# sqlp/sedumi

Hardware: AMD Instinct MI355X
Metric: IPM iters/sec (ADA' form+factor+solve) (higher is better)
Workload: dtype f64; 1 GPU; control07.mat: examples/control07.mat (BASELINE.json configs[1]), m=666, nnz(At)=107940, nnz(ADA')=443556, nnz(L)=222111; unit = getada1+2+3, blkchol, 4x(fwblkslv,./d,bwblkslv); parallelism=single GPU

## Files before the change

### sedumi_amd/csrc/sdm_ada.hip

```cpp
#include "sdm_plan.h"
#include <algorithm>
#include <cmath>
#include <cstdlib>

namespace sdm {

void ada_build(sdm_plan *P, sdm_int N, sdm_int m, const sdm_int *Ajc, const sdm_int *Air, const double *Apr,
               const sdm_int *Ajc_psd, sdm_int lpN, sdm_int lorN, const sdm_int *lorNL, sdm_int sdpN,
               sdm_int rsdpN, const sdm_int *sdpNL, const sdm_int *qblkstart, const sdm_int *psd_blkstart,
               const sdm_int *Qjc, const sdm_int *Qir, const sdm_int *ADAjc, const sdm_int *ADAir) {
  AdaPlan &A = P->ada;
  A.N = N; A.m = m; A.nnzA = Ajc[m]; A.lpN = lpN; A.lorN = lorN; A.sdpN = sdpN; A.rsdpN = rsdpN;
  A.ic_n.release(); A.ufac.release();
  if (A.nnzA >= (sdm_int)1 << 31 || N >= (sdm_int)1 << 31) throw std::runtime_error("At too large for 32-bit row indices");
  (void)lorNL;
  A.nlq = sdpN > 0 ? psd_blkstart[0] : N;
  if (lorN > 0 && qblkstart[lorN] != A.nlq && sdpN > 0) throw std::runtime_error("qblkstart / psd_blkstart mismatch");
  {
    std::vector<int> code((size_t)A.nlq, -1);
    for (sdm_int r = lpN; r < lpN + lorN && r < A.nlq; r++) code[r] = (int)(-2 - (r - lpN));
    for (sdm_int k = 0; k < lorN; k++)
      for (sdm_int r = qblkstart[k]; r < qblkstart[k + 1] && r < A.nlq; r++) code[r] = (int)k;
    A.dsqr_code.upload(code);
  }
// ... 443 lines not shown
  const int task = order ? order[blockIdx.x] : blockIdx.x + task0;
  const int n = T.t_n[task], nslot = T.t_nslot[task], ulen = T.t_ulen[task];
  const int herm = T.t_herm[task];
  const int64_t slot0 = T.t_slotptr[task], tend = T.t_end[task];
  const double *D = udsqr + T.t_udoff[task];
  const double *Di = D + (int64_t)n * n;
  const int *U = T.u_pos + T.t_uoff[task];
  double *z = zbuf + T.t_zoff[task];
  const int64_t rowbase = T.psd_start[T.t_blk[task]];
  const int tid = threadIdx.x, bs = blockDim.x;
  const int wave = tid >> 6, lane = tid & 63, nw = bs >> 6;
  int CC = ldsY / (n * (herm ? 4 : 2)); if (CC < 1) CC = 1; if (CC > nslot) CC = nslot;
  double *Yi = Y + (int64_t)CC * n;
  double *Dl = Y + (int64_t)(herm ? 2 : 1) * CC * n;
  double *Dli = Dl + (int64_t)CC * n;
  double *nzx = Y + ldsY;
  int *nzr = (int *)(nzx + nzcap);
  __shared__ int scol[256];
  const int64_t nzb = T.s_nzptr[slot0];
  const bool staged = tend - nzb <= nzcap;
  if (staged)
    for (int64_t u = nzb + tid; u < tend; u += bs) { nzx[u - nzb] = T.Apr[u]; nzr[u - nzb] = (int)(T.Air[u] - rowbase); }
  constexpr int S1_TREG = 6;
  int rreg[S1_TREG], creg[S1_TREG];
  double zreg[S1_TREG];
  const int nreg = herm ? 0 : min(ulen, S1_TREG * bs);
  if (!herm) {
#pragma unroll
    for (int k = 0; k < S1_TREG; k++) {
      const int q = U[min(tid + k * bs, max(ulen - 1, 0))];
      creg[k] = q / n; rreg[k] = q - creg[k] * n; zreg[k] = 0.0;
    }
  }
  for (int c0 = 0; c0 < nslot; c0 += CC) {
    const int cc = min(CC, nslot - c0);
    for (int t = tid; t < min(cc, 256); t += bs) scol[t] = T.s_col[slot0 + c0 + t];
    __syncthreads();
    const bool flat = cc < nw;
    for (int t = flat ? 0 : wave; t < cc; t += flat ? 1 : nw) {
      const int64_t sb = T.s_nzptr[slot0 + c0 + t];
      const int64_t se = (c0 + t + 1 < nslot) ? T.s_nzptr[slot0 + c0 + t + 1] : tend;
      const int sc = t < 256 ? scol[t] : T.s_col[slot0 + c0 + t];
      const int part = sc >= n ? 1 : 0, col = sc - part * n;
      const int sub0 = part * n * n + col * n;
      if (!herm && !flat && n <= 256) {
        double a4[4] = {0.0, 0.0, 0.0, 0.0}, d4[4];
        int i4[4];
#pragma unroll
        for (int k = 0; k < 4; k++) { i4[k] = min(lane + 64 * k, n - 1); d4[k] = D[(int64_t)col * n + i4[k]]; }
        for (int64_t u = sb; u < se; u++) {
          const int rx = (staged ? nzr[u - nzb] : (int)(T.Air[u] - rowbase)) - sub0;
          const double x = staged ? nzx[u - nzb] : T.Apr[u];
          double dr[4];
#pragma unroll
          for (int k = 0; k < 4; k++) dr[k] = D[(int64_t)rx * n + i4[k]];
#pragma unroll
          for (int k = 0; k < 4; k++) a4[k] += x * dr[k];
        }
#pragma unroll
        for (int k = 0; k < 4; k++)
          if (lane + 64 * k < n) { Y[t * n + lane + 64 * k] = a4[k]; Dl[t * n + lane + 64 * k] = d4[k]; }
        continue;
      }
      for (int i = flat ? tid : lane; i < n; i += flat ? bs : 64) {
        double ar = 0.0, ai = 0.0;
        for (int64_t u = sb; u < se; u++) {
          const int rx = (staged ? nzr[u - nzb] : (int)(T.Air[u] - rowbase)) - sub0;
          const double x = staged ? nzx[u - nzb] : T.Apr[u], dr = D[(int64_t)rx * n + i];
          if (!herm) ar += x * dr;
          else {
            const double di = Di[(int64_t)rx * n + i];
            if (part) { ar -= x * di; ai += x * dr; } else { ar += x * dr; ai += x * di; }
          }
        }
        Y[t * n + i] = ar;
        Dl[t * n + i] = D[(int64_t)col * n + i];
        if (herm) { Yi[t * n + i] = ai; Dli[t * n + i] = -Di[(int64_t)col * n + i]; }
      }
    }
    __syncthreads();
    if (!herm) {
      double sreg[S1_TREG];
#pragma unroll
      for (int k = 0; k < S1_TREG; k++) sreg[k] = 0.0;
#pragma unroll 1
      for (int t = 0; t < cc; t++) {
        const double *Yt = Y + t * n, *Dt = Dl + t * n;
#pragma unroll
        for (int k = 0; k < S1_TREG; k++) sreg[k] += Yt[rreg[k]] * Dt[creg[k]] + Yt[creg[k]] * Dt[rreg[k]];
      }
#pragma unroll
      for (int k = 0; k < S1_TREG; k++) zreg[k] += sreg[k] / 2;
    }
    for (int u = nreg + tid; u < ulen; u += bs) {
      int q = U[u];
      const int zpart = q >= n * n ? 1 : 0;
      q -= zpart * n * n;
      const int c = q / n, r = q - c * n;
      double v;
      if (!herm) {
        double a1 = 0.0, a2 = 0.0;
        for (int t = 0; t < cc; t++) {
          a1 += Y[t * n + r] * Dl[t * n + c];
          a2 += Y[t * n + c] * Dl[t * n + r];
        }
        v = (a1 + a2) / 2;
      } else {
        double rrc = 0.0, irc = 0.0, rcr = 0.0, icr = 0.0;
        for (int t = 0; t < cc; t++) {
          const double drc = Dl[t * n + c], dic = Dli[t * n + c], drr = Dl[t * n + r], dir = Dli[t * n + r];
          const double yr_r = Y[t * n + r], yi_r = Yi[t * n + r], yr_c = Y[t * n + c], yi_c = Yi[t * n + c];
          rrc += yr_r * drc - yi_r * dic; irc += yr_r * dic + yi_r * drc;
          rcr += yr_c * drr - yi_c * dir; icr += yr_c * dir + yi_c * drr;
        }
        v = zpart ? (irc - icr) / 2 : (rrc + rcr) / 2;
      }
      if (c0 == 0) z[u] = v; else z[u] += v;
    }
    __syncthreads();
  }
  if (!herm && R2.ada && ulen <= S1_TREG * bs) {
    double *zl = Y;
#pragma unroll
    for (int k = 0; k < S1_TREG; k++) if (tid + k * bs < ulen) zl[tid + k * bs] = zreg[k];
    __syncthreads();
    const int j = R2.t_col[task], kblk = T.t_blk[task];
    const int ipj = R2.invperm ? R2.invperm[j] : 0;
    for (int64_t e = R2.ADAjc[j] + tid; e < R2.ADAjc[j + 1]; e += bs) {
      const int i = R2.ADAir[e];
      if (R2.invperm && R2.invperm[i] > ipj) continue;
      double acc = 0.0, aabs = 0.0;
      int64_t p = R2.Ajc_psd[i];
      const int64_t pe = R2.Ajc[i + 1];
      for (; p + 4 <= pe; p += 4) {
        double x[4]; int b[4], u[4];
#pragma unroll
        for (int q = 0; q < 4; q++) { x[q] = R2.Apr[p + q]; b[q] = R2.Ablk[p + q]; u[q] = R2.Aupos[p + q]; }
#pragma unroll
        for (int q = 0; q < 4; q++) if (b[q] == kblk) { const double term = x[q] * zl[u[q]]; acc += term; aabs += fabs(term); }
      }
      for (; p < pe; p++) if (R2.Ablk[p] == kblk) { const double term = R2.Apr[p] * zl[R2.Aupos[p]]; acc += term; aabs += fabs(term); }
      const double base = R2.ada[e];
      R2.ada[e] = base + acc;
      if (i == j) R2.absd[j] = base + aabs;
    }
    return;
  }
  if (!herm) {
#pragma unroll
    for (int k = 0; k < S1_TREG; k++) if (tid + k * bs < ulen) z[tid + k * bs] = zreg[k];
  }
}

__global__ void __launch_bounds__(64 * S1_WAVES, 4)
k_psd_stage1_mfma(Stage1Tab T, const double *udsqr, double *zbuf, int task0, const int *order, double *zero_ptr, long long zero_n) {
  SDM_DYN_SMEM(smem);
  for (long long i = (long long)blockIdx.x * blockDim.x + threadIdx.x; i < zero_n; i += (long long)gridDim.x * blockDim.x) zero_ptr[i] = 0.0;
  const int task = order ? order[blockIdx.x] : blockIdx.x + task0;
  const int n = T.t_n[task], nslot = T.t_nslot[task], ulen = T.t_ulen[task];
  const int np = (n + 15) & ~15, nt = np >> 4, ntile = nt * nt;
  double *Yl = (double *)smem;
  double *Dl = Yl + S1_KC * np;
  double *Zl = (double *)smem;
  const int64_t slot0 = T.t_slotptr[task], tend = T.t_end[task];
  const double *D = udsqr + T.t_udoff[task];
  double *z = zbuf + T.t_zoff[task];
  const int64_t rowbase = T.psd_start[T.t_blk[task]];
  const int tid = threadIdx.x, bs = blockDim.x;
  const int wave = SDM_UNIFORM_INT(tid >> 6), lane = tid & 63, nw = bs >> 6;
  const int li = lane & 15, lk = lane >> 4;
  sdm_double4 acc[S1_MAXT];
  for (int x = 0; x < S1_MAXT; x++) for (int r = 0; r < 4; r++) acc[x][r] = 0.0;
  __shared__ double nzx[S1_NZ];
  __shared__ int nzr[S1_NZ];
  __shared__ int sbeg[S1_MAXN + 1], scol[S1_MAXN];
  SDM_PHASE_BEGIN();
  const int64_t nzb = T.s_nzptr[slot0];
  const bool staged = tend - nzb <= S1_NZ && nslot <= S1_MAXN;
  if (staged) {
    for (int64_t u = nzb + tid; u < tend; u += bs) { nzx[u - nzb] = T.Apr[u]; nzr[u - nzb] = (int)(T.Air[u] - rowbase); }
    for (int t = tid; t <= nslot; t += bs) sbeg[t] = (int)((t < nslot ? T.s_nzptr[slot0 + t] : tend) - nzb);
    for (int t = tid; t < nslot; t += bs) scol[t] = T.s_col[slot0 + t];
  }
  __syncthreads();
  SDM_PHASE(0);
  for (int c0 = 0; c0 < nslot; c0 += S1_KC) {
    const int cc = min(S1_KC, nslot - c0);
    for (int t = wave; t < S1_KC; t += nw) {
      if (t < cc) {
        int sb, se, col;
        if (staged) { sb = sbeg[c0 + t]; se = sbeg[c0 + t + 1]; col = scol[c0 + t]; }
        else {
          sb = (int)(T.s_nzptr[slot0 + c0 + t] - nzb);
          se = (int)(((c0 + t + 1 < nslot) ? T.s_nzptr[slot0 + c0 + t + 1] : tend) - nzb);
          col = T.s_col[slot0 + c0 + t];
        }
        for (int i = lane; i < np; i += 64) {
          double a = 0.0;
          if (i < n) {
            if (staged) {
              int u = sb;
              for (; u + 4 <= se; u += 4) {
                const double d0 = D[(int64_t)(nzr[u] - col * n) * n + i], d1 = D[(int64_t)(nzr[u + 1] - col * n) * n + i];
                const double d2 = D[(int64_t)(nzr[u + 2] - col * n) * n + i], d3 = D[(int64_t)(nzr[u + 3] - col * n) * n + i];
                a += nzx[u] * d0; a += nzx[u + 1] * d1; a += nzx[u + 2] * d2; a += nzx[u + 3] * d3;
              }
              for (; u < se; u++) a += nzx[u] * D[(int64_t)(nzr[u] - col * n) * n + i];
            } else {
              for (int64_t u = nzb + sb; u < nzb + se; u++) a += T.Apr[u] * D[(int64_t)((int)(T.Air[u] - rowbase) - col * n) * n + i];
            }
          }
          Yl[t * np + i] = a;
          Dl[t * np + i] = i < n ? D[(int64_t)col * n + i] : 0.0;
        }
      } else {
        for (int i = lane; i < np; i += 64) { Yl[t * np + i] = 0.0; Dl[t * np + i] = 0.0; }
      }
    }
    SDM_PHASE(1);
    __syncthreads();
    SDM_PHASE(2);
    for (int x = 0; x < S1_MAXT; x++) {
      const int tile = wave + x * nw;
      if (tile < ntile) {
        const int I = tile / nt, J = tile - I * nt;
#pragma unroll 4
        for (int q = 0; q < S1_KC / 4; q++) {
          const double a = Yl[(4 * q + lk) * np + I * 16 + li];
          const double b = Dl[(4 * q + lk) * np + J * 16 + li];
          acc[x] = SDM_MFMA_F64_16x16x4(a, b, acc[x]);
        }
      }
    }
    SDM_PHASE(3);
    __syncthreads();
    SDM_PHASE(4);
  }
  for (int x = 0; x < S1_MAXT; x++) {
    const int tile = wave + x * nw;
    if (tile < ntile) {
      const int I = tile / nt, J = tile - I * nt;
      for (int r = 0; r < 4; r++) Zl[(I * 16 + lk + 4 * r) * np + J * 16 + li] = acc[x][r];
    }
  }
  __syncthreads();
  SDM_PHASE(5);
  const int *RC = T.u_rc + T.t_uoff[task];
  for (int u0 = 0; u0 < ulen; u0 += 8 * bs) {
    int rc[8];
#pragma unroll
    for (int x = 0; x < 8; x++) rc[x] = RC[min(u0 + x * bs + tid, ulen - 1)];
#pragma unroll
    for (int x = 0; x < 8; x++) {
      const int u = u0 + x * bs + tid;
      const int r = rc[x] >> 16, c = rc[x] & 0xffff;
      if (u < ulen) z[u] = (Zl[r * np + c] + Zl[c * np + r]) / 2;
    }
  }
  SDM_PHASE(6);
#if defined(SDM_PHASES) && !defined(SDM_EMU)
  if (tid == 0) { atomicAdd(&sdm_phase_acc[30], 1ull); if (n > 40) atomicAdd(&sdm_phase_acc[31], 1ull); }
#endif
}

__global__ void __launch_bounds__(256)
k_psd_stage2(double *ada, double *absd, const int64_t *ADAjc, const int *ADAir, const int64_t *Ajc,
             const int64_t *Ajc_psd, const double *Apr, const int *Ablk, const int *Aupos,
             const int64_t *c_taskptr, const int *t_blk, const int64_t *t_zoff, const int64_t *c_zlen, const double *zbuf,
             const int *invperm, int nblk, int thread_per_row, int jbase, int zlds) {
  SDM_DYN_SMEM(smem);
  long long *zo = (long long *)smem;
  double *zl = (double *)(zo + nblk);
  const int j = blockIdx.x + jbase;
  const int tid = threadIdx.x, bs = blockDim.x;
  const int64_t tb0 = c_taskptr[j], te0 = c_taskptr[j + 1];
  const bool jhas = te0 > tb0;
  const int64_t z0 = jhas ? t_zoff[tb0] : 0;
  const int64_t zlen = c_zlen[j];
  for (int k = tid; k < nblk; k += bs) zo[k] = -1;
  __syncthreads();
  for (int64_t t = tb0 + tid; t < te0; t += bs) zo[t_blk[t]] = t_zoff[t] - z0;
  const bool staged = thread_per_row && jhas && zlen <= zlds;
  if (staged)
    for (int64_t u = tid; u < zlen; u += bs) zl[u] = zbuf[z0 + u];
  __syncthreads();
  const double *zsrc = staged ? zl : zbuf + z0;
  const int ipj = invperm ? invperm[j] : 0;
  if (thread_per_row) {
    for (int64_t e = ADAjc[j] + tid; e < ADAjc[j + 1]; e += bs) {
      const int i = ADAir[e];
      if (invperm && invperm[i] > ipj) continue;
      double acc = 0.0, aabs = 0.0;
      if (jhas) {
        int64_t t = Ajc_psd[i];
        const int64_t te = Ajc[i + 1];
        for (; t + 4 <= te; t += 4) {
          double x[4]; int b[4], u[4];
#pragma unroll
          for (int q = 0; q < 4; q++) { x[q] = Apr[t + q]; b[q] = Ablk[t + q]; u[q] = Aupos[t + q]; }
#pragma unroll
          for (int q = 0; q < 4; q++) {
            const long long off = zo[b[q]];
            if (off >= 0) { const double term = x[q] * zsrc[off + u[q]]; acc += term; aabs += fabs(term); }
          }
        }
        for (; t < te; t++) {
          const long long off = zo[Ablk[t]];
          if (off >= 0) { const double term = Apr[t] * zsrc[off + Aupos[t]]; acc += term; aabs += fabs(term); }
        }
      }
      const double base = ada[e];
      ada[e] = base + acc;
      if (i == j) absd[j] = jhas ? base + aabs : 0.0;
    }
  } else {
    const int wave = tid >> 6, lane = tid & 63, nw = bs >> 6;
    for (int64_t e = ADAjc[j] + wave; e < ADAjc[j + 1]; e += nw) {
      const int i = ADAir[e];
      if (invperm && invperm[i] > ipj) continue;
      double acc = 0.0, aabs = 0.0;
      if (jhas)
        for (int64_t t = Ajc_psd[i] + lane; t < Ajc[i + 1]; t += 64) {
          const long long off = zo[Ablk[t]];
          if (off >= 0) { const double term = Apr[t] * zsrc[off + Aupos[t]]; acc += term; aabs += fabs(term); }
        }
      for (int off = 32; off > 0; off >>= 1) { acc += __shfl_down(acc, off); aabs += __shfl_down(aabs, off); }
      if (lane == 0) {
        const double base = ada[e];
        ada[e] = base + acc;
        if (i == j) absd[j] = jhas ? base + aabs : 0.0;
      }
    }
  }
}

constexpr int S1_DIRECT_MAXNZ = 2;
constexpr int DIRECT_JB = 8;
__global__ void __launch_bounds__(256)
k_psd_direct_cols(double *ada, double *absd, const int64_t *ADAjc, const int64_t *Ajc, const int64_t *Ajc_psd, const double *Apr,
                  const int *Air, const int *Ablk, const int64_t *c_taskptr, const int *t_blk, const int *t_n, const int64_t *t_udoff,
                  const int64_t *t_slotptr, const int64_t *s_nzptr, const int64_t *t_end, const int64_t *psd_start, const double *udsqr,
                  int nblk, int jbase, int jend, int m, int base_zero) {
  SDM_DYN_SMEM(smem);
  const int per_i = 2 * nblk + 2 * S1_DIRECT_MAXNZ * nblk + 2, per_ll = 2 * nblk, per_d = S1_DIRECT_MAXNZ * nblk;
  int *bn_all = (int *)smem;
  long long *ll_all = (long long *)(bn_all + DIRECT_JB * (per_i + (per_i & 1)));
  double *bx_all = (double *)(ll_all + DIRECT_JB * per_ll);
  __shared__ int jhas_s[DIRECT_JB];
  int *bnk = (int *)(bx_all + DIRECT_JB * per_d);
  const int tid = threadIdx.x, bs = blockDim.x;
  const int j0 = jbase + DIRECT_JB * blockIdx.x;
  const int stride_i = per_i + (per_i & 1);
  for (int jj = 0; jj < DIRECT_JB; jj++) {
    int *bn = bn_all + jj * stride_i, *bnz = bn + nblk, *brc = bnz + nblk;
    long long *bud = ll_all + jj * per_ll, *bst = bud + nblk;
    double *bx = bx_all + jj * per_d;
    for (int k = tid; k < nblk; k += bs) {
      bn[k] = 0; bnz[k] = 0; bst[k] = psd_start[k]; bud[k] = 0;
      for (int w = 0; w < S1_DIRECT_MAXNZ; w++) { brc[(k * S1_DIRECT_MAXNZ + w) * 2] = 0; brc[(k * S1_DIRECT_MAXNZ + w) * 2 + 1] = 0; bx[k * S1_DIRECT_MAXNZ + w] = 0.0; }
    }
  }
  __syncthreads();
  for (int jj = 0; jj < DIRECT_JB; jj++) {
    const int j = j0 + jj;
    if (j >= jend) { if (tid == 0) jhas_s[jj] = 0; continue; }
    int *bn = bn_all + jj * stride_i, *bnz = bn + nblk, *brc = bnz + nblk;
    long long *bud = ll_all + jj * per_ll;
    double *bx = bx_all + jj * per_d;
    const int64_t tb0 = c_taskptr[j], te0 = c_taskptr[j + 1];
    if (tid == 0) jhas_s[jj] = te0 > tb0 ? 1 : 0;
    for (int64_t t = tb0 + tid; t < te0; t += bs) {
      const int k = t_blk[t], n = t_n[t];
      const int64_t u0 = s_nzptr[t_slotptr[t]], u1 = t_end[t];
      bn[k] = n; bud[k] = t_udoff[t]; bnz[k] = (int)(u1 - u0);
      for (int64_t u = u0; u < u1 && u - u0 < S1_DIRECT_MAXNZ; u++) {
        const int q = (int)(Air[u] - psd_start[k]);
        brc[(k * S1_DIRECT_MAXNZ + (int)(u - u0)) * 2] = q % n; brc[(k * S1_DIRECT_MAXNZ + (int)(u - u0)) * 2 + 1] = q / n;
        bx[k * S1_DIRECT_MAXNZ + (int)(u - u0)] = Apr[u];
      }
    }
  }
  __syncthreads();
  for (int k = tid; k < nblk; k += bs) {
    int nk = 0;
    for (int jj = 0; jj < DIRECT_JB; jj++) nk = max(nk, (bn_all + jj * stride_i)[k]);
    bnk[k] = nk;
  }
  __syncthreads();
  const long long *bst0 = ll_all + nblk;
  const int rows_per = ((m + (int)gridDim.y - 1) / (int)gridDim.y + 1) & ~1;
  const int i_end = min(m, ((int)blockIdx.y + 1) * rows_per);
  for (int i = (int)blockIdx.y * rows_per + tid; i < i_end; i += bs) {
    double acc[DIRECT_JB], aabs[DIRECT_JB];
#pragma unroll
    for (int jj = 0; jj < DIRECT_JB; jj++) { acc[jj] = 0.0; aabs[jj] = 0.0; }
    for (int64_t p = Ajc_psd[i]; p < Ajc[i + 1]; p++) {
      const int k = Ablk[p];
      const int n = bnk[k];
      if (n == 0) continue;
      const int q = (int)(Air[p] - bst0[k]);
      const double xp = Apr[p];
      const int c = q / n, r = q - c * n;
#pragma unroll
      for (int jj = 0; jj < DIRECT_JB; jj++) {
        const int *bn = bn_all + jj * stride_i;
        if (bn[k] == 0 || !jhas_s[jj]) continue;
        const int *bnz = bn + nblk, *brc = bnz + nblk;
        const double *D = udsqr + (ll_all + jj * per_ll)[k];
        const double *bx = bx_all + jj * per_d;
// ... 252 lines not shown
      }
    }
    __syncthreads();
  }
}

__global__ void k_symmetrize(double *out, const double *in, const int64_t *ADAjc, const int *ADAir, const int *adaT, int m) {
  int j = blockIdx.x;
  if (j < (m / 128) * 128) { const int r = j & 127; j = (j & ~127) + (r & 7) * 16 + (r >> 3); }
  for (int64_t e = ADAjc[j] + threadIdx.x; e < ADAjc[j + 1]; e += blockDim.x) {
    const int i = ADAir[e];
    double v = in[e];
    if (i != j) { const int et = adaT[e]; if (et >= 0) v += in[et]; }
    out[e] = v;
  }
}
__global__ void k_diag(double *absd, const double *ada, const int64_t *ADAjc, const int *ADAir, int m) {
  const int j = blockIdx.x * blockDim.x + threadIdx.x;
  if (j >= m) return;
  int64_t lo = ADAjc[j], hi = ADAjc[j + 1];
  const int64_t ce = hi;
  while (lo < hi) { const int64_t mid = (lo + hi) >> 1; if (ADAir[mid] < j) lo = mid + 1; else hi = mid; }
  absd[j] = (lo < ce && ADAir[lo] == j) ? ada[lo] : 0.0;
}

void ada_zero_flush(sdm_plan *P) {
  AdaPlan &A = P->ada;
  if (A.zero_ptr && A.zero_n > 0) SDM_HIP_CHECK(hipMemsetAsync(A.zero_ptr, 0, (size_t)A.zero_n * sizeof(double), P->stream));
  A.zero_ptr = nullptr; A.zero_n = 0;
}
void ada_lq(sdm_plan *P, double *ada, const int *d_invperm, bool accumulate) {
  AdaPlan &A = P->ada;
  if (A.col1 <= A.col0) return;
  if (A.nnz_lq == 0 && !accumulate && !d_invperm) {
    const sdm_int e0 = P->ada_jc[A.col0], e1 = P->ada_jc[A.col1];
    ada_zero_flush(P);
    if (e1 > e0) { A.zero_ptr = ada + e0; A.zero_n = (long long)(e1 - e0); }
    if (!A.zero_defer) ada_zero_flush(P);
    return;
  }
  if (A.nlq > 0)
    SDM_KLAUNCH(P, k_dsqr, dim3((unsigned)((A.nlq + 255) / 256)), dim3(256), 0, A.dsqr.p, A.dsqr_code.p, A.dl.p, A.ddet.p, (int)A.nlq);
  if (A.lq_dense) {
    const int m = (int)A.m, nt = (m + TILE - 1) / TILE;
    SDM_KLAUNCH(P, k_gram_tile, dim3(nt * (nt + 1) / 2, A.gram_split), dim3(256), 0, A.Alq_d.p, A.dsqr.p, (int)A.nlq, m, A.gram_split,
                A.gram_part.p);
    SDM_KLAUNCH(P, k_gram_scatter, dim3((unsigned)(A.col1 - A.col0)), dim3(128), 0, ada, A.d_ADAjc.p, A.d_ADAir.p, A.gram_part.p,
                A.gram_split, m, d_invperm, accumulate ? 1 : 0, (int)A.col0);
    return;
  }
  if (A.lq_maxcol <= 256)
    SDM_KLAUNCH(P, k_ada_spdot<16>, dim3((unsigned)(A.col1 - A.col0)), dim3(256), (size_t)SPDOT_CAP * 12, ada, A.d_ADAjc.p, A.d_ADAir.p, A.d_Ajc.p, A.d_Ajc_psd.p,
               A.d_Air.p, A.d_Apr.p, A.dsqr.p, d_invperm, accumulate ? 1 : 0, (int)A.col0, SPDOT_CAP);
  else
    SDM_KLAUNCH(P, k_ada_spdot<64>, dim3((unsigned)(A.col1 - A.col0)), dim3(256), (size_t)SPDOT_CAP * 12, ada, A.d_ADAjc.p, A.d_ADAir.p, A.d_Ajc.p, A.d_Ajc_psd.p,
               A.d_Air.p, A.d_Apr.p, A.dsqr.p, d_invperm, accumulate ? 1 : 0, (int)A.col0, SPDOT_CAP);
}
void ada_datq(sdm_plan *P) {
  AdaPlan &A = P->ada;
  if (A.lorN == 0 || A.nnzQ == 0) return;
  SDM_KLAUNCH(P, k_datq, dim3((unsigned)A.m), dim3(128), 0, A.qpr.p, A.d_Qjc.p, A.d_Qir.p, A.d_Ajc.p, A.d_Ajc_psd.p, A.d_Air.p, A.d_Apr.p,
              A.q1.p, A.q2.p, A.d_qblk.p, (int)A.lpN);
}
void ada_q(sdm_plan *P, double *ada, const int *d_invperm, bool accumulate) {
  AdaPlan &A = P->ada;
  if (A.lorN == 0 || A.nnzQ == 0 || A.col1 <= A.col0) return;
  ada_zero_flush(P);
  if (A.q_dense) {
    const int m = (int)A.m, nt = (m + TILE - 1) / TILE;
    SDM_HIP_CHECK(hipMemsetAsync(A.Q_d.p, 0, (size_t)A.lorN * (size_t)m * sizeof(double), P->stream));
    SDM_KLAUNCH(P, k_q_densify, dim3((unsigned)((A.nnzQ + 255) / 256)), dim3(256), 0, A.Q_d.p, A.qpr.p, A.q_dst.p, (int64_t)A.nnzQ);
    SDM_KLAUNCH(P, k_gram_tile, dim3(nt * (nt + 1) / 2, A.gram_split), dim3(256), 0, A.Q_d.p, (const double *)nullptr, (int)A.lorN, m,
                A.gram_split, A.gram_part.p);
    SDM_KLAUNCH(P, k_gram_scatter, dim3((unsigned)(A.col1 - A.col0)), dim3(128), 0, ada, A.d_ADAjc.p, A.d_ADAir.p, A.gram_part.p,
                A.gram_split, m, d_invperm, accumulate ? 1 : 0, (int)A.col0);
    return;
  }
  if (A.q_maxcol <= 256)
    SDM_KLAUNCH(P, k_ada_spdot<16>, dim3((unsigned)(A.col1 - A.col0)), dim3(256), (size_t)SPDOT_CAP * 12, ada, A.d_ADAjc.p, A.d_ADAir.p, A.d_Qjc.p, A.d_Qjc.p + 1,
               A.d_Qir.p, A.qpr.p, (const double *)nullptr, d_invperm, accumulate ? 1 : 0, (int)A.col0, SPDOT_CAP);
  else
    SDM_KLAUNCH(P, k_ada_spdot<64>, dim3((unsigned)(A.col1 - A.col0)), dim3(256), (size_t)SPDOT_CAP * 12, ada, A.d_ADAjc.p, A.d_ADAir.p, A.d_Qjc.p, A.d_Qjc.p + 1,
               A.d_Qir.p, A.qpr.p, (const double *)nullptr, d_invperm, accumulate ? 1 : 0, (int)A.col0, SPDOT_CAP);
}
bool ada_lq_q(sdm_plan *P, double *ada) {
  AdaPlan &A = P->ada;
  const int m = (int)A.m;
  if (!(A.lq_dense && A.q_dense && A.q_src.n && A.col0 == 0 && A.col1 == A.m && A.lorN > 0 && A.nnzQ > 0)) return false;
  const int64_t nq = (int64_t)A.lorN * m, nprep = std::max<int64_t>(nq, A.nlq);
  const int nt = (m + TILE - 1) / TILE;
  SDM_KLAUNCH(P, k_lq_q_prep, dim3((unsigned)((nprep + 255) / 256)), dim3(256), 0, A.dsqr.p, A.dsqr_code.p, A.dl.p, A.ddet.p, (int)A.nlq,
              A.Q_d.p, A.qpr.p, A.q_src.p, nq);
  SDM_KLAUNCH(P, k_gram_tile, dim3(nt * (nt + 1) / 2, A.gram_split), dim3(256), 0, A.Alq_d.p, A.dsqr.p, (int)A.nlq, m, A.gram_split,
              A.gram_part.p, A.Q_d.p, (int)A.lorN);
  SDM_KLAUNCH(P, k_gram_scatter, dim3((unsigned)m), dim3(128), 0, ada, A.d_ADAjc.p, A.d_ADAir.p, A.gram_part.p, A.gram_split, m,
              (const int *)nullptr, 0, 0, A.sdpN == 0 ? P->absd.p : (double *)nullptr);
  return true;
}
void ada_psd(sdm_plan *P, double *ada, const int *d_invperm, bool sym_input, bool absd_done) {
  AdaPlan &A = P->ada;
  hipStream_t st = P->stream;
  const int m = (int)A.m;
  if (A.sdpN == 0 || sym_input || A.col1 <= A.col0) ada_zero_flush(P);
  if (A.sdpN == 0) {
    if (sym_input) {
      SDM_KLAUNCH(P, k_symmetrize, dim3(m), dim3(128), 0, A.symtmp.p, ada, A.d_ADAjc.p, A.d_ADAir.p, A.d_ADAT.p, m);
      SDM_HIP_CHECK(hipMemcpyAsync(ada, A.symtmp.p, A.symtmp.n * sizeof(double), hipMemcpyDeviceToDevice, st));
    }
    if (!absd_done) SDM_KLAUNCH(P, k_diag, dim3((m + 255) / 256), dim3(256), 0, P->absd.p, ada, A.d_ADAjc.p, A.d_ADAir.p, m);
    return;
  }
  if (A.col1 <= A.col0) return;
  const int ncols = (int)(A.col1 - A.col0), jbase = (int)A.col0;
  const int task0 = (int)A.h_taskptr[A.col0], ntask = (int)(A.h_taskptr[A.col1] - A.h_taskptr[A.col0]);
  const size_t direct_lds = (size_t)(2 * A.sdpN + 2 * S1_DIRECT_MAXNZ * A.sdpN + 2) * sizeof(int) + (size_t)(2 * A.sdpN) * sizeof(long long) +
                            (size_t)(S1_DIRECT_MAXNZ * A.sdpN) * sizeof(double);
  const bool direct = A.thread_per_row && !A.ell_ok && A.sdpN == A.rsdpN && A.s1_maxnz <= S1_DIRECT_MAXNZ && direct_lds <= S1_DIRECT_LDS_MAX;
  const bool direct_zero = direct && !sym_input && !d_invperm && A.zero_ptr == ada + P->ada_jc[A.col0] &&
                           A.zero_n == (long long)(P->ada_jc[A.col1] - P->ada_jc[A.col0]);
  if (direct_zero) { A.zero_ptr = nullptr; A.zero_n = 0; }
  if (direct || ntask <= 0 || !(A.maxn <= S1_MAXN && A.sdpN == A.rsdpN)) ada_zero_flush(P);
  if (direct) {
    if (sym_input) {
      SDM_KLAUNCH(P, k_symmetrize, dim3(m), dim3(128), 0, A.symtmp.p, ada, A.d_ADAjc.p, A.d_ADAir.p, A.d_ADAT.p, m);
      SDM_HIP_CHECK(hipMemcpyAsync(ada, A.symtmp.p, A.symtmp.n * sizeof(double), hipMemcpyDeviceToDevice, st));
    }
    const int nb = (int)A.sdpN;
    const size_t lds = direct_lds;
    const size_t lds_cols = (size_t)DIRECT_JB * (direct_lds + 16) + (size_t)A.sdpN * sizeof(int);
    if (!d_invperm && (int64_t)(P->ada_jc[A.col1] - P->ada_jc[A.col0]) == (int64_t)ncols * m && lds_cols <= S1_DIRECT_LDS_MAX) {
      const int ysplit = std::max(1, std::min(16, (int)((m + 511) / 512)));
      SDM_KLAUNCH(P, k_psd_direct_cols, dim3((ncols + DIRECT_JB - 1) / DIRECT_JB, ysplit), dim3(256), lds_cols, ada, P->absd.p, A.d_ADAjc.p, A.d_Ajc.p, A.d_Ajc_psd.p, A.d_Apr.p,
                  A.d_Air.p, A.d_Ablk.p, A.c_taskptr.p, A.t_blk.p, A.t_n.p, A.t_udoff.p, A.t_slotptr.p, A.s_nzptr.p, A.t_end.p, A.d_psd_start.p, A.udsqr.p,
                  nb, jbase, jbase + ncols, m, direct_zero ? 1 : 0);
      SDM_HIP_CHECK(hipGetLastError());
      return;
    }
    SDM_KLAUNCH(P, k_psd_direct, dim3(ncols), dim3(256), lds, ada, P->absd.p, A.d_ADAjc.p, A.d_ADAir.p, A.d_Ajc.p, A.d_Ajc_psd.p, A.d_Apr.p, A.d_Air.p,
                A.d_Ablk.p, A.c_taskptr.p, A.t_blk.p, A.t_n.p, A.t_udoff.p, A.t_slotptr.p, A.s_nzptr.p, A.t_end.p, A.d_psd_start.p, A.udsqr.p,
                d_invperm, nb, jbase, direct_zero ? 1 : 0);
    SDM_HIP_CHECK(hipGetLastError());
    return;
  }
  bool stage1_cleared_all = false;
  if (ntask > 0) {
    Stage1Tab T;
    T.t_n = A.t_n.p; T.t_nslot = A.t_nslot.p; T.t_ulen = A.t_ulen.p; T.t_herm = A.t_herm.p; T.s_col = A.s_col.p;
    T.u_pos = A.u_pos.p; T.u_rc = A.u_rc.p; T.Air = A.d_Air.p; T.t_slotptr = A.t_slotptr.p; T.t_udoff = A.t_udoff.p; T.t_uoff = A.t_uoff.p;
    T.t_zoff = A.t_zoff.p; T.t_end = A.t_end.p; T.s_nzptr = A.s_nzptr.p; T.Apr = A.d_Apr.p; T.t_blk = A.t_blk.p;
    T.psd_start = A.d_psd_start.p;
#ifndef SDM_EMU
    SDM_HIP_CHECK(hipFuncSetAttribute((const void *)k_psd_stage1, hipFuncAttributeMaxDynamicSharedMemorySize, (int)A.stage1_lds));
#endif
    if (A.maxn <= S1_MAXN && A.sdpN == A.rsdpN) {
      const int np = (A.maxn + 15) & ~15;
      const size_t lds = (size_t)std::max(2 * S1_KC * np, np * np) * sizeof(double);
#ifndef SDM_EMU
      if (lds > 48 * 1024) SDM_HIP_CHECK(hipFuncSetAttribute((const void *)k_psd_stage1_mfma, hipFuncAttributeMaxDynamicSharedMemorySize, (int)lds));
#endif
      double *zp = A.zero_ptr; const long long zn = A.zero_n;
      A.zero_ptr = nullptr; A.zero_n = 0;
      stage1_cleared_all = zp == ada + P->ada_jc[A.col0] && zn == (long long)(P->ada_jc[A.col1] - P->ada_jc[A.col0]);
      SDM_KLAUNCH(P, k_psd_stage1_mfma, dim3((unsigned)ntask), dim3(64 * S1_WAVES), lds, T, A.udsqr.p, A.zbuf.p, task0,
                  (ntask == (int)A.ntask) ? (const int *)A.t_order.p : (const int *)nullptr, zp, zn);
    } else
    {
      const size_t one = (size_t)(A.sdpN > A.rsdpN ? 4 : 2) * (size_t)A.maxn * sizeof(double);
      const size_t ldsy = std::max(one, std::min(A.stage1_lds, (size_t)S1_GEN_LDS));
      const int nzcap = (int)std::min<int64_t>(S1_NZ, (A.s1_maxnz + 1) & ~(int64_t)1);
      const size_t lds = ldsy + (size_t)nzcap * (sizeof(double) + sizeof(int));
#ifndef SDM_EMU
      SDM_HIP_CHECK(hipFuncSetAttribute((const void *)k_psd_stage1, hipFuncAttributeMaxDynamicSharedMemorySize, (int)lds));
#endif
      const bool ride = A.one_task_per_col && A.thread_per_row && !A.ell_ok && A.sdpN == A.rsdpN && A.s1_maxulen <= 6 * 512 &&
                        (int64_t)A.s1_maxulen * (int64_t)sizeof(double) <= (int64_t)ldsy;
      Stage2Ride R2 = {};
      if (ride) {
        if (sym_input) {
          SDM_KLAUNCH(P, k_symmetrize, dim3(m), dim3(128), 0, A.symtmp.p, ada, A.d_ADAjc.p, A.d_ADAir.p, A.d_ADAT.p, m);
          SDM_HIP_CHECK(hipMemcpyAsync(ada, A.symtmp.p, A.symtmp.n * sizeof(double), hipMemcpyDeviceToDevice, st));
        }
        SDM_HIP_CHECK(hipMemsetAsync(P->absd.p + jbase, 0, (size_t)ncols * sizeof(double), st));
        R2.ada = ada; R2.absd = P->absd.p; R2.ADAjc = A.d_ADAjc.p; R2.Ajc = A.d_Ajc.p; R2.Ajc_psd = A.d_Ajc_psd.p; R2.ADAir = A.d_ADAir.p;
        R2.Ablk = A.d_Ablk.p; R2.Aupos = A.d_Aupos.p; R2.t_col = A.t_col.p; R2.invperm = d_invperm; R2.Apr = A.d_Apr.p;
      }
      SDM_KLAUNCH(P, k_psd_stage1, dim3((unsigned)ntask), dim3(512), lds, T, A.udsqr.p, A.zbuf.p, (int)(ldsy / sizeof(double)), task0, nzcap, R2,
                  (ntask == (int)A.ntask && A.t_order_xcd.n == (size_t)ntask) ? (const int *)A.t_order_xcd.p : (const int *)nullptr);
      if (ride) { SDM_HIP_CHECK(hipGetLastError()); return; }
    }
  }
  if (sym_input) {
    SDM_KLAUNCH(P, k_symmetrize, dim3(m), dim3(128), 0, A.symtmp.p, ada, A.d_ADAjc.p, A.d_ADAir.p, A.d_ADAT.p, m);
    SDM_HIP_CHECK(hipMemcpyAsync(ada, A.symtmp.p, A.symtmp.n * sizeof(double), hipMemcpyDeviceToDevice, st));
  }
  if (A.ell_ok) {
    auto lds_of = [&](int jb) { return (size_t)jb * (size_t)A.zmax * sizeof(double); };
#define SDM_STAGE2_ELL(JB)                                                                                              \
    do {                                                                                                                 \
      const size_t lds = lds_of(JB);                                                                                    \
      SDM_STAGE2_ATTR(JB, lds);                                                                                         \
      SDM_KLAUNCH(P, k_psd_stage2_ell<JB>, dim3((ncols + JB - 1) / JB, gsplit), dim3(64 * ELL_WAVES), lds, ada, P->absd.p, A.d_ADAjc.p, A.d_ADAir.p, \
                  A.d_Ajc.p, A.d_Ajc_psd.p, A.d_Apr.p, A.d_Ablk.p, A.d_Aupos.p, A.c_taskptr.p, A.t_blk.p, A.t_ulen.p,    \
                  A.t_zoff.p, A.zbuf.p, A.d_uoff.p, A.g_row.p, A.g_len.p, A.g_off.p, A.g_val.p, A.g_bu.p, A.ell_ng, d_invperm, \
                  (int)A.zmax, m, jbase, jbase + ncols, A.ell_pos.p, sym ? (const int *)A.ell_order.p : (const int *)nullptr,     \
                  A.d_Azpos.p, A.t_zdst.p, stage1_cleared_all && !sym_input ? 1 : 0,                                             \
                  sym ? (const long long *)A.cdp64.p : (const long long *)A.cdc64.p, sym ? (const int *)A.cdp32.p : (const int *)A.cdc32.p); \
    } while (0)
#ifndef SDM_EMU
#define SDM_STAGE2_ATTR(JB, lds) if ((lds) > 48 * 1024) SDM_HIP_CHECK(hipFuncSetAttribute((const void *)k_psd_stage2_ell<JB>, hipFuncAttributeMaxDynamicSharedMemorySize, (int)(lds)))
#else
#define SDM_STAGE2_ATTR(JB, lds) (void)(lds)
#endif
    const bool sym = A.ell_full && !d_invperm && jbase == 0 && ncols == m;
    const int gsplit = sym ? 3 : 1;
    if (lds_of(4) <= 64 * 1024 && m >= 1024) SDM_STAGE2_ELL(4);
    else if (lds_of(2) <= 64 * 1024 && m >= 512) SDM_STAGE2_ELL(2);
    else SDM_STAGE2_ELL(1);
#undef SDM_STAGE2_ELL
#undef SDM_STAGE2_ATTR
    SDM_HIP_CHECK(hipGetLastError());
    return;
  }
  {
    const int64_t zl = (A.thread_per_row && A.zmaxj * 8 <= 64 * 1024) ? A.zmaxj : 0;
    const size_t lds = (size_t)A.sdpN * 8 + (size_t)zl * 8;
#ifndef SDM_EMU
    if (lds > 48 * 1024) SDM_HIP_CHECK(hipFuncSetAttribute((const void *)k_psd_stage2, hipFuncAttributeMaxDynamicSharedMemorySize, (int)lds));
#endif
    SDM_KLAUNCH(P, k_psd_stage2, dim3(ncols), dim3(256), lds, ada, P->absd.p, A.d_ADAjc.p, A.d_ADAir.p, A.d_Ajc.p,
               A.d_Ajc_psd.p, A.d_Apr.p, A.d_Ablk.p, A.d_Aupos.p, A.c_taskptr.p, A.t_blk.p, A.t_zoff.p, A.c_zlen.p, A.zbuf.p,
               d_invperm, (int)A.sdpN, A.thread_per_row ? 1 : 0, jbase, (int)zl);
  }
  SDM_HIP_CHECK(hipGetLastError());
}

}

#if defined(SDM_PHASES) && !defined(SDM_EMU)
extern "C" int sdm_debug_phases_ada(unsigned long long *out32, int reset) {
  if (out32 && hipMemcpyFromSymbol(out32, HIP_SYMBOL(sdm_phase_acc), 32 * sizeof(unsigned long long)) != hipSuccess) return 1;
  if (reset) { unsigned long long z[32] = {0}; if (hipMemcpyToSymbol(HIP_SYMBOL(sdm_phase_acc), z, sizeof(z)) != hipSuccess) return 1; }
  return 0;
}
#endif
```

### sedumi_amd/csrc/sdm_plan.h

```cpp
#pragma once
#include "../../include/sedumi_hip.h"
#include "sdm_rt.h"
#include <mutex>
#include <string>
#include <vector>

namespace sdm {

constexpr int NB = 64;
constexpr int TILE = 64;
constexpr int UTP = 72;
constexpr int S1_MAXN = 96;
constexpr int S1_KC = 48;
constexpr int S1_WAVES = 8;
constexpr int S1_NZ = 1536;
constexpr int S1_MAXT = ((S1_MAXN / 16) * (S1_MAXN / 16) + S1_WAVES - 1) / S1_WAVES;
constexpr int S1_GEN_LDS = 74 * 1024;
constexpr int ELL_WAVES = 8;
constexpr int SOLVE_LDS_MAX = 3072;
constexpr int FUSE_MAX_TILES = 1 << 20;
constexpr int SBW_MIN = 256;
constexpr int SBW_MAX = 2048;
constexpr int SINV_MAXLEV = 4;
constexpr int SPREP_NCNT = 2 + 2 * SINV_MAXLEV;
constexpr int SROWS = 16;
#ifndef SDM_SW
#define SDM_SW 8
#endif
constexpr int SW = SDM_SW;
constexpr int LDL_THREADS = 512;
constexpr int PANEL_THREADS = 256;
constexpr int ROWS_BATCH = 16 * (PANEL_THREADS / 64);
constexpr int TRSM_ROWS = 128;
#ifndef SDM_MFMA_MIN_ROWS
#define SDM_MFMA_MIN_ROWS 48
#endif
constexpr int MFMA_MIN_ROWS = SDM_MFMA_MIN_ROWS;
constexpr int CHK = 16;
constexpr int64_t ASM_FULL_MAX = 4 << 20;
constexpr int FRONT_MAXT = 64;
constexpr int FRONT_XCNT_OFF = 2 * FRONT_MAXT + FRONT_MAXT * FRONT_MAXT;
constexpr int FRONT_CNT = FRONT_XCNT_OFF + FRONT_MAXT * FRONT_MAXT;
constexpr int FRONT_POOL = 1;
constexpr int PANEL_RB = (LDL_THREADS / 64) * NB * 17;
constexpr size_t PANEL_LDS = (size_t)(NB * (NB + 1) + PANEL_RB) * sizeof(double);
constexpr size_t PANEL_LDS_RIDE = std::max(PANEL_LDS, (size_t)4 * NB * UTP * sizeof(double));
constexpr int FRONT_CV_OFF = NB * (NB + 1) + (LDL_THREADS / 64) * NB * 17;
constexpr size_t FRONT_LDS = (size_t)(FRONT_CV_OFF + NB * TILE) * sizeof(double);
static_assert(PANEL_RB >= NB * NB && PANEL_RB >= (NB - CHK) * TRSM_ROWS && TRSM_ROWS == 16 * (LDL_THREADS / 64) && ROWS_BATCH <= TRSM_ROWS, "panel LDS layout");

template <class T>
struct DevBuf {
  T *p = nullptr;
  size_t n = 0;
  DevBuf() = default;
  DevBuf(const DevBuf &) = delete;
  DevBuf &operator=(const DevBuf &) = delete;
  DevBuf(DevBuf &&o) noexcept : p(o.p), n(o.n) { o.p = nullptr; o.n = 0; }
  DevBuf &operator=(DevBuf &&o) noexcept { if (this != &o) { release(); p = o.p; n = o.n; o.p = nullptr; o.n = 0; } return *this; }
  ~DevBuf() { release(); }
  void release() {
    if (p) (void)hipFree(p);
    p = nullptr; n = 0;
  }
  void alloc(size_t count) {
    release();
    n = count;
    SDM_HIP_CHECK(hipMalloc((void **)&p, (count ? count : 1) * sizeof(T)));
  }
  void upload(const std::vector<T> &h) {
    alloc(h.size());
    if (!h.empty()) SDM_HIP_CHECK(hipMemcpy(p, h.data(), h.size() * sizeof(T), hipMemcpyHostToDevice));
  }
  void upload(const T *h, size_t count) {
    alloc(count);
    if (count) SDM_HIP_CHECK(hipMemcpy(p, h, count * sizeof(T), hipMemcpyHostToDevice));
  }
};

struct PanelCtx {
  double *lb; const double *ubp; int *pivstat; double *pivval; double *colbuf; const double *ada; const int *asm_src; const int64_t *Ljc;
  int mtot, pad;
};

struct HostFlag {
  int *host = nullptr;
  HostFlag() = default;
  HostFlag(const HostFlag &) = delete;
  HostFlag &operator=(const HostFlag &) = delete;
  HostFlag(HostFlag &&o) noexcept : host(o.host) { o.host = nullptr; }
  HostFlag &operator=(HostFlag &&o) noexcept { if (this != &o) { if (host) (void)hipHostFree(host); host = o.host; o.host = nullptr; } return *this; }
  ~HostFlag() { if (host) (void)hipHostFree(host); }
  void ensure() {
    if (host) return;
    SDM_HIP_CHECK(hipHostMalloc((void **)&host, 4 * sizeof(int), 0));
    for (int i = 0; i < 4; i++) host[i] = 0;
  }
  int *dev() {
    ensure();
    void *d = nullptr;
    SDM_HIP_CHECK(hipHostGetDevicePointer(&d, host, 0));
    return (int *)d;
  }
};

struct PinnedInts {
  int *p = nullptr; size_t n = 0;
  PinnedInts() = default;
  PinnedInts(const PinnedInts &) = delete;
  PinnedInts &operator=(const PinnedInts &) = delete;
  ~PinnedInts() { if (p) (void)hipHostFree(p); }
  void ensure(size_t count) {
    if (count <= n) return;
    if (p) (void)hipHostFree(p);
    p = nullptr; n = 0;
    SDM_HIP_CHECK(hipHostMalloc((void **)&p, (count ? count : 1) * sizeof(int), 0));
    n = count;
  }
};

struct LevelLaunch {
  int level, panel;
  int nactive;
  int maxrows;
  int maxtiles;
  int lasttiles;
  int q0;
  int ride_wgs;
};

struct SolveLevel {
  int nfronts = 0, maxns = 0, maxms = 0, nsb = 0;
  bool children = false;
  bool below = false;
  std::vector<int> slabs_fw;
};

struct CholPlan {
  sdm_int m = 0, nsuper = 0, nnzL = 0, nnzADA = 0;
  int nlevels = 0;
  int64_t fsize = 0, wsize = 0, tsize = 0;
  int maxms = 0, maxns = 0;
  std::vector<sdm_int> Ljc, perm;
  std::vector<int> sn_first, sn_ns, sn_ms, sn_ld, sn_parent, sn_level;
  std::vector<int64_t> sn_foff, sn_xl, sn_woff, sn_roff, sn_toff;
  std::vector<int> childptr, childlist, levptr, levlist, lev_T;
  std::vector<char> sn_active;
  double pars_canceltol = 0, pars_maxu = 0, pars_abstol = 0; int pars_use_absd = 0;
  bool begun = false;
  std::vector<LevelLaunch> launches;
  std::vector<int> lev_first_launch;
  DevBuf<int> d_first, d_ns, d_ms, d_ld, d_parent, d_childptr, d_childlist, d_levlist, d_lindx, d_relidx, d_perm;
  DevBuf<int64_t> d_foff, d_xl, d_woff, d_roff, d_toff, d_asm_dst, d_asm_dstT, d_Ljc;
  DevBuf<int> d_asm_src;
  DevBuf<double> fronts, frontsT, wvec, colbuf, d, dsolve, lb, pivval, ub;
  DevBuf<int> pivstat;
  DevBuf<int> diag_cnt;
  DevBuf<int> d_asm_fsrc;
  DevBuf<int> front_cnt;
  DevBuf<int> d_fslot;
  std::vector<char> lev_persist;
  std::vector<int> lev_maxT;
  std::vector<int> lev_ntw;
  DevBuf<int> upd_cnt;
  DevBuf<double> panelrec;
  DevBuf<PanelCtx> panel_ctx;
  PanelCtx panel_ctx_host = {};
  HostFlag tmo;
// ... 281 lines not shown
```

Measured before the change: 2647 IPM iters/s.

## Rework PSD stage1 MFMA kernel LDS sizing, flatten fill loop, trim K padding

The MFMA stage-1 kernel now sizes its nonzero staging buffers dynamically from the actual max nnz instead of fixed static arrays, shrinks the K chunk from 48 to 32, and raises the launch-bounds occupancy hint. The Y/D fill loop is flattened across all threads with reciprocal division instead of per-wave row loops, padding is zeroed once, and MFMA iterations stop at the rounded-up actual chunk width. The Z tile uses an odd leading dimension to avoid LDS bank conflicts. These aim to cut LDS footprint and wasted work and raise occupancy, at the cost of more chunk iterations and possible register pressure.

```diff
diff --git a/sedumi_amd/csrc/sdm_ada.hip b/sedumi_amd/csrc/sdm_ada.hip
--- a/sedumi_amd/csrc/sdm_ada.hip
+++ b/sedumi_amd/csrc/sdm_ada.hip
@@ -619,8 +619,8 @@
   }
 }
 
-__global__ void __launch_bounds__(64 * S1_WAVES, 4)
-k_psd_stage1_mfma(Stage1Tab T, const double *udsqr, double *zbuf, int task0, const int *order, double *zero_ptr, long long zero_n) {
+__global__ void __launch_bounds__(64 * S1_WAVES, 3 * S1_WAVES / 4)
+k_psd_stage1_mfma(Stage1Tab T, const double *udsqr, double *zbuf, int ldsY, int nzcap, int task0, const int *order, double *zero_ptr, long long zero_n) {
   SDM_DYN_SMEM(smem);
   for (long long i = (long long)blockIdx.x * blockDim.x + threadIdx.x; i < zero_n; i += (long long)gridDim.x * blockDim.x) zero_ptr[i] = 0.0;
   const int task = order ? order[blockIdx.x] : blockIdx.x + task0;
@@ -629,6 +629,7 @@
   double *Yl = (double *)smem;
   double *Dl = Yl + S1_KC * np;
   double *Zl = (double *)smem;
+  const int ldz = n | 1;
   const int64_t slot0 = T.t_slotptr[task], tend = T.t_end[task];
   const double *D = udsqr + T.t_udoff[task];
   double *z = zbuf + T.t_zoff[task];
@@ -636,14 +637,16 @@
   const int tid = threadIdx.x, bs = blockDim.x;
   const int wave = SDM_UNIFORM_INT(tid >> 6), lane = tid & 63, nw = bs >> 6;
   const int li = lane & 15, lk = lane >> 4;
+  const int rcpn = ((1 << 20) + n - 1) / n;
+  static_assert(S1_KC * S1_MAXN * S1_MAXN < (1 << 20) && S1_KC % 4 == 0, "k_psd_stage1_mfma: reciprocal division, four slots per MFMA step");
   sdm_double4 acc[S1_MAXT];
   for (int x = 0; x < S1_MAXT; x++) for (int r = 0; r < 4; r++) acc[x][r] = 0.0;
-  __shared__ double nzx[S1_NZ];
-  __shared__ int nzr[S1_NZ];
+  double *nzx = (double *)smem + ldsY;
+  int *nzr = (int *)(nzx + nzcap);
   __shared__ int sbeg[S1_MAXN + 1], scol[S1_MAXN];
   SDM_PHASE_BEGIN();
   const int64_t nzb = T.s_nzptr[slot0];
-  const bool staged = tend - nzb <= S1_NZ && nslot <= S1_MAXN;
+  const bool staged = tend - nzb <= nzcap && nslot <= S1_MAXN;
   if (staged) {
     for (int64_t u = nzb + tid; u < tend; u += bs) { nzx[u - nzb] = T.Apr[u]; nzr[u - nzb] = (int)(T.Air[u] - rowbase); }
     for (int t = tid; t <= nslot; t += bs) sbeg[t] = (int)((t < nslot ? T.s_nzptr[slot0 + t] : tend) - nzb);
@@ -651,39 +654,36 @@
   }
   __syncthreads();
   SDM_PHASE(0);
+  for (int t = wave; t < S1_KC; t += nw)
+    if (lane < np - n) { Yl[t * np + n + lane] = 0.0; Dl[t * np + n + lane] = 0.0; }
   for (int c0 = 0; c0 < nslot; c0 += S1_KC) {
-    const int cc = min(S1_KC, nslot - c0);
-    for (int t = wave; t < S1_KC; t += nw) {
-      if (t < cc) {
-        int sb, se, col;
-        if (staged) { sb = sbeg[c0 + t]; se = sbeg[c0 + t + 1]; col = scol[c0 + t]; }
-        else {
-          sb = (int)(T.s_nzptr[slot0 + c0 + t] - nzb);
-          se = (int)(((c0 + t + 1 < nslot) ? T.s_nzptr[slot0 + c0 + t + 1] : tend) - nzb);
-          col = T.s_col[slot0 + c0 + t];
-        }
-        for (int i = lane; i < np; i += 64) {
-          double a = 0.0;
-          if (i < n) {
-            if (staged) {
-              int u = sb;
-              for (; u + 4 <= se; u += 4) {
-                const double d0 = D[(int64_t)(nzr[u] - col * n) * n + i], d1 = D[(int64_t)(nzr[u + 1] - col * n) * n + i];
-                const double d2 = D[(int64_t)(nzr[u + 2] - col * n) * n + i], d3 = D[(int64_t)(nzr[u + 3] - col * n) * n + i];
-                a += nzx[u] * d0; a += nzx[u + 1] * d1; a += nzx[u + 2] * d2; a += nzx[u + 3] * d3;
-              }
-              for (; u < se; u++) a += nzx[u] * D[(int64_t)(nzr[u] - col * n) * n + i];
-            } else {
-              for (int64_t u = nzb + sb; u < nzb + se; u++) a += T.Apr[u] * D[(int64_t)((int)(T.Air[u] - rowbase) - col * n) * n + i];
-            }
-          }
-          Yl[t * np + i] = a;
-          Dl[t * np + i] = i < n ? D[(int64_t)col * n + i] : 0.0;
-        }
+    const int cc = min(S1_KC, nslot - c0), kq = (cc + 3) & ~3;
+    for (int e = tid; e < cc * n; e += bs) {
+      const int t = (e * rcpn) >> 20, i = e - t * n;
+      int sb, se, col;
+      if (staged) { sb = sbeg[c0 + t]; se = sbeg[c0 + t + 1]; col = scol[c0 + t]; }
+      else {
+        sb = (int)(T.s_nzptr[slot0 + c0 + t] - nzb);
+        se = (int)(((c0 + t + 1 < nslot) ? T.s_nzptr[slot0 + c0 + t + 1] : tend) - nzb);
+        col = T.s_col[slot0 + c0 + t];
+      }
+      double a = 0.0;
+      if (staged) {
+        int u = sb;
+        for (; u + 4 <= se; u += 4) {
+          const double d0 = D[(int64_t)(nzr[u] - col * n) * n + i], d1 = D[(int64_t)(nzr[u + 1] - col * n) * n + i];
+          const double d2 = D[(int64_t)(nzr[u + 2] - col * n) * n + i], d3 = D[(int64_t)(nzr[u + 3] - col * n) * n + i];
+          a += nzx[u] * d0; a += nzx[u + 1] * d1; a += nzx[u + 2] * d2; a += nzx[u + 3] * d3;
+        }
+        for (; u < se; u++) a += nzx[u] * D[(int64_t)(nzr[u] - col * n) * n + i];
       } else {
-        for (int i = lane; i < np; i += 64) { Yl[t * np + i] = 0.0; Dl[t * np + i] = 0.0; }
-      }
-    }
+        for (int64_t u = nzb + sb; u < nzb + se; u++) a += T.Apr[u] * D[(int64_t)((int)(T.Air[u] - rowbase) - col * n) * n + i];
+      }
+      Yl[t * np + i] = a;
+      Dl[t * np + i] = D[(int64_t)col * n + i];
+    }
+    for (int t = cc + wave; t < kq; t += nw)
+      for (int i = lane; i < n; i += 64) { Yl[t * np + i] = 0.0; Dl[t * np + i] = 0.0; }
     SDM_PHASE(1);
     __syncthreads();
     SDM_PHASE(2);
@@ -691,12 +691,17 @@
       const int tile = wave + x * nw;
       if (tile < ntile) {
         const int I = tile / nt, J = tile - I * nt;
-#pragma unroll 4
-        for (int q = 0; q < S1_KC / 4; q++) {
-          const double a = Yl[(4 * q + lk) * np + I * 16 + li];
-          const double b = Dl[(4 * q + lk) * np + J * 16 + li];
-          acc[x] = SDM_MFMA_F64_16x16x4(a, b, acc[x]);
-        }
+        int npo = np; SDM_PIN(npo);
+        const double *Ya = Yl + lk * npo + I * 16 + li, *Db = Dl + lk * npo + J * 16 + li;
+        int q = 0;
+        for (; q + 4 <= kq / 4; q += 4) {
+          double a[4], b[4];
+#pragma unroll
+          for (int k = 0; k < 4; k++) { a[k] = Ya[4 * (q + k) * npo]; b[k] = Db[4 * (q + k) * npo]; }
+#pragma unroll
+          for (int k = 0; k < 4; k++) acc[x] = SDM_MFMA_F64_16x16x4(a[k], b[k], acc[x]);
+        }
+        for (; q < kq / 4; q++) acc[x] = SDM_MFMA_F64_16x16x4(Ya[4 * q * npo], Db[4 * q * npo], acc[x]);
       }
     }
     SDM_PHASE(3);
@@ -707,7 +712,8 @@
     const int tile = wave + x * nw;
     if (tile < ntile) {
       const int I = tile / nt, J = tile - I * nt;
-      for (int r = 0; r < 4; r++) Zl[(I * 16 + lk + 4 * r) * np + J * 16 + li] = acc[x][r];
+      for (int r = 0; r < 4; r++)
+        if (I * 16 + lk + 4 * r < n && J * 16 + li < n) Zl[(I * 16 + lk + 4 * r) * ldz + J * 16 + li] = acc[x][r];
     }
   }
   __syncthreads();
@@ -721,7 +727,7 @@
     for (int x = 0; x < 8; x++) {
       const int u = u0 + x * bs + tid;
       const int r = rc[x] >> 16, c = rc[x] & 0xffff;
-      if (u < ulen) z[u] = (Zl[r * np + c] + Zl[c * np + r]) / 2;
+      if (u < ulen) z[u] = (Zl[r * ldz + c] + Zl[c * ldz + r]) / 2;
     }
   }
   SDM_PHASE(6);
@@ -1280,22 +1286,22 @@
 #ifndef SDM_EMU
     SDM_HIP_CHECK(hipFuncSetAttribute((const void *)k_psd_stage1, hipFuncAttributeMaxDynamicSharedMemorySize, (int)A.stage1_lds));
 #endif
+    const int nzcap = s1_nzcap(A.s1_maxnz);
     if (A.maxn <= S1_MAXN && A.sdpN == A.rsdpN) {
-      const int np = (A.maxn + 15) & ~15;
-      const size_t lds = (size_t)std::max(2 * S1_KC * np, np * np) * sizeof(double);
+      const int ldsy = s1_mfma_ldsy(A.maxn);
+      const size_t lds = s1_mfma_lds(A.maxn, A.s1_maxnz);
 #ifndef SDM_EMU
       if (lds > 48 * 1024) SDM_HIP_CHECK(hipFuncSetAttribute((const void *)k_psd_stage1_mfma, hipFuncAttributeMaxDynamicSharedMemorySize, (int)lds));
 #endif
       double *zp = A.zero_ptr; const long long zn = A.zero_n;
       A.zero_ptr = nullptr; A.zero_n = 0;
       stage1_cleared_all = zp == ada + P->ada_jc[A.col0] && zn == (long long)(P->ada_jc[A.col1] - P->ada_jc[A.col0]);
-      SDM_KLAUNCH(P, k_psd_stage1_mfma, dim3((unsigned)ntask), dim3(64 * S1_WAVES), lds, T, A.udsqr.p, A.zbuf.p, task0,
+      SDM_KLAUNCH(P, k_psd_stage1_mfma, dim3((unsigned)ntask), dim3(64 * S1_WAVES), lds, T, A.udsqr.p, A.zbuf.p, ldsy, nzcap, task0,
                   (ntask == (int)A.ntask) ? (const int *)A.t_order.p : (const int *)nullptr, zp, zn);
     } else
     {
       const size_t one = (size_t)(A.sdpN > A.rsdpN ? 4 : 2) * (size_t)A.maxn * sizeof(double);
       const size_t ldsy = std::max(one, std::min(A.stage1_lds, (size_t)S1_GEN_LDS));
-      const int nzcap = (int)std::min<int64_t>(S1_NZ, (A.s1_maxnz + 1) & ~(int64_t)1);
       const size_t lds = ldsy + (size_t)nzcap * (sizeof(double) + sizeof(int));
 #ifndef SDM_EMU
       SDM_HIP_CHECK(hipFuncSetAttribute((const void *)k_psd_stage1, hipFuncAttributeMaxDynamicSharedMemorySize, (int)lds));
diff --git a/sedumi_amd/csrc/sdm_plan.h b/sedumi_amd/csrc/sdm_plan.h
--- a/sedumi_amd/csrc/sdm_plan.h
+++ b/sedumi_amd/csrc/sdm_plan.h
@@ -11,9 +11,12 @@
 constexpr int TILE = 64;
 constexpr int UTP = 72;
 constexpr int S1_MAXN = 96;
-constexpr int S1_KC = 48;
+constexpr int S1_KC = 32;
 constexpr int S1_WAVES = 8;
 constexpr int S1_NZ = 1536;
+constexpr int s1_nzcap(int64_t maxnz) { return (int)(((maxnz + 1) & ~(int64_t)1) < S1_NZ ? ((maxnz + 1) & ~(int64_t)1) : S1_NZ); }
+constexpr int s1_mfma_ldsy(int maxn) { return 2 * S1_KC * ((maxn + 15) & ~15) > maxn * (maxn | 1) ? 2 * S1_KC * ((maxn + 15) & ~15) : maxn * (maxn | 1); }
+constexpr size_t s1_mfma_lds(int maxn, int64_t maxnz) { return (size_t)s1_mfma_ldsy(maxn) * sizeof(double) + (size_t)s1_nzcap(maxnz) * (sizeof(double) + sizeof(int)); }
 constexpr int S1_MAXT = ((S1_MAXN / 16) * (S1_MAXN / 16) + S1_WAVES - 1) / S1_WAVES;
 constexpr int S1_GEN_LDS = 74 * 1024;
 constexpr int ELL_WAVES = 8;
```

After: 2815 IPM iters/s, median of 6. +6.3%, better.
